# apache/brpc

Hardware: NVIDIA H100
Metric: echo QPS, 1 KB baidu_std (higher is better)
Workload: dtype u8

## Files before the change

### brpc_b200/csrc/b2_api.cu

```cuda
#include <cuda_runtime.h>
#include <dlfcn.h>
#include <stdio.h>
#include <time.h>
#include <stdlib.h>
#include <string.h>
#include <algorithm>
#include <mutex>
#include <string>
#include <unordered_map>
#include <vector>
#include "b2_kernels.cuh"
#include "b2_h2.cuh"

using namespace b2;

static thread_local char g_err[512] = "";
static void set_err(const char* fmt, const char* a = "", const char* b = "") { snprintf(g_err, sizeof g_err, fmt, a, b); }

#define CU(call)                                                                          \
    do {                                                                                  \
        cudaError_t e_ = (call);                                                          \
        if (e_ != cudaSuccess) { set_err("%s: %s", #call, cudaGetErrorString(e_)); return B2_E_CUDA; } \
    } while (0)

namespace {
constexpr int kMaxStages = 16;
constexpr uint32_t kSmallBytes = 128 << 10;
constexpr uint32_t kSmallRuns = 512, kSmallMsgs = 1024;
constexpr size_t kSmallBlock = 64 + kSmallRuns * 32 + kSmallMsgs * (64 + 16) + (kSmallBytes + kSmallMsgs * 80 + 4096);
constexpr uint32_t kSecEvents = 64, kSecMsgs = kSecEvents + kSmallMsgs * 80, kSecCtrl = kSecMsgs + kSmallMsgs * 32,
                   kSecRunCtrl = kSecCtrl + 3 * kStreamCtrlMax * kSmallMsgs, kSecOut = kSecRunCtrl + kSmallRuns * 8;
struct Stage { const char* name; cudaEvent_t ev; };
}

struct b2_ctx {
    b2_options opt;
    DevConfig cfg;
    std::vector<DevMethod> methods;
    uint8_t* d_bytes = nullptr; b2_run* d_runs = nullptr; uint32_t* d_run_tile_base = nullptr;
    TileRec* d_tiles = nullptr; uint32_t* d_tile_base = nullptr; uint32_t* d_tile_scratch = nullptr; uint32_t* d_tile_spec = nullptr; b2_run_status* d_run_status = nullptr;
    uint32_t* d_frame_off = nullptr; uint32_t* d_frame_run = nullptr; b2_msg_desc* d_msgs = nullptr; MsgAux* d_aux = nullptr; PackJob* d_jobs = nullptr; uint32_t* d_slow_idx = nullptr; uint8_t* d_heads = nullptr;
    uint32_t* d_slot = nullptr; uint32_t* d_scan_tmp = nullptr; uint8_t* d_resp = nullptr; uint8_t* d_unz = nullptr; uint16_t* d_snappy_tab = nullptr; HpackState* d_hpack = nullptr; H2Conn* d_h2 = nullptr; H2Stream* d_h2_streams = nullptr; uint8_t* d_h2_slots = nullptr; uint32_t h2_max_conns = B2_H2_MAX_CONNS, h2_pending = B2_H2_MAX_PENDING, h2_stream_bytes = B2_H2_STREAM_BYTES; uint64_t h2_last_in = 0, h2_last_out = 0;
    uint32_t* d_frame_row = nullptr; uint4* d_rows = nullptr;
    std::vector<uint8_t> h2_gunzip; uint8_t* d_h2_gz_merge = nullptr;
    uint8_t* ring_slots = nullptr; volatile uint32_t* ring_ctl = nullptr; uint32_t* d_ring_ticket = nullptr; cudaStream_t ring_stream = nullptr;
    uint32_t ring_next = 1, ring_stride = 0, ring_off_runs = 0, ring_off_in = 0, ring_off_out = 0; bool ring_collected[8] = { true, true, true, true, true, true, true, true };
    const void* ring_bytes[8] = {}; const void* ring_pin_base = nullptr; unsigned long long ring_pin_dev = 0; uint64_t ring_launches = 0;
    bool st_ring = false; StreamPass sp_ring = {}; uint8_t* d_st_ring = nullptr; uint32_t ring_off_st = 0, ring_next_wait = 1, st_view_ticket = 0;
    bool h2_ring = false; uint32_t h2r_max_bytes = 0, h2r_msg_cap = 0, h2r_out_cap = 0, h2r_replies_cap = 0;
    uint32_t h2r_off_args = 0, h2r_off_rs = 0, h2r_off_msgs = 0, h2r_off_spans = 0, h2r_off_out = 0, h2r_off_replies = 0;
    ulonglong2* d_iov = nullptr; b2_iovec* h_iov = nullptr; const void* host_bytes = nullptr;
    uint4* d_refs = nullptr; b2_resp_ref* h_refs = nullptr; int input_mode = B2_INPUT_COPY, resp_mode = B2_RESP_COPY; const uint8_t* pull_bytes = nullptr; uint32_t small_off_refs = 0;
    uint32_t* d_crc_adv = nullptr; unsigned long long* d_counters = nullptr; uint32_t* d_totals = nullptr; DevMethod* d_methods = nullptr;
    size_t meta_tile_off = 0; uint32_t max_tiles = 0; uint32_t n_sms = 132; bool use_tma_pack = true; uint32_t stage_mask = 7;
    StreamPass sp = {}; bool has_streams = false, stream_armed = false, stream_ran = false, stream_valid = false;
    uint32_t st_max = 0, st_open = 0; std::vector<long long> st_keys; std::vector<uint8_t> st_state; std::vector<uint32_t> st_pool, st_pool_free;
    void* d_st_block[10] = {}; void* h_st_mapped[5] = {}; uint32_t* h_st_cnts = nullptr; uint8_t* h_st_out = nullptr; uint8_t* h_st_ctl = nullptr; uint8_t* d_st_ctl = nullptr;
    b2_stream_msg* h_st_msgs = nullptr; b2_stream_event* h_st_events = nullptr; uint8_t* h_st_ctrl = nullptr; uint32_t* h_st_run_ctrl = nullptr;
    cudaEvent_t st_ev[6] = {};
    const uint8_t* st_input = nullptr;
    void* d_sw[4] = {}; size_t sw_have[4] = {}; SwRec* h_sw_recs = nullptr; size_t h_sw_have = 0; uint32_t* h_sw_cnts = nullptr;
    cudaEvent_t sw_ev[8] = {}; bool sw_ran = false;
    b2_run_status* h_run_status = nullptr; b2_msg_desc* h_msgs = nullptr; uint8_t* h_resp = nullptr;
    uint32_t* h_totals = nullptr; uint32_t* h_run_tile_base = nullptr;
    uint32_t n_runs = 0, n_tiles = 0, nbytes = 0, max_run_tiles = 0; uint64_t covered = 0;
    bool uploaded = false, executed = false;
    cudaStream_t stream = nullptr;
    cudaEvent_t ev[kMaxStages + 1];
    const char* stage_names[kMaxStages];
    int n_stages = 0;
    float last_kernel_ms = 0.f; uint32_t last_launches = 0;
    cudaEvent_t ev_first = nullptr, ev_last = nullptr; bool first_pending = true;
    bool profile_stages = false; bool allow_small = true; bool use_fused = true; bool fused_last = false; bool slow_heavy = false;
    bool adaptive_tile = false; bool dense = false; uint32_t avg_frame = 0;
    uint8_t* d_meta = nullptr; uint8_t* h_meta = nullptr;
    uint8_t* d_small = nullptr; uint8_t* h_small = nullptr;
    bool small = false, small_copy_queued = false, use_fused_small = true; uint32_t small_msgs = 0, small_resp = 0, small_off_rs = 0, small_off_msgs = 0, small_off_resp = 0, small_total = 0;
};

static void input_overwritten(b2_ctx* c) { if (c->st_input == c->d_bytes) c->st_input = nullptr; }

static uint32_t g_crc_tab_host[256];
static void crc_table_init() {
    for (uint32_t i = 0; i < 256; i++) {
        uint32_t c = i;
        for (int k = 0; k < 8; k++) c = (c & 1) ? (c >> 1) ^ 0x82f63b78u : (c >> 1);
        g_crc_tab_host[i] = c;
    }
}

extern "C" const char* b2_last_error(void) { return g_err; }
extern "C" const char* b2_version(void) { return "brpc_b200 0.1 (sm_90a)"; }

namespace {
struct BlockPool {
    std::mutex mu;
    static constexpr size_t kSmall = 8192, kSlab = 4u << 20;
    std::vector<uint8_t*> slabs; std::vector<void*> small_free;
    std::unordered_map<void*, int> large_class;
    std::vector<void*> large_free[40];
    uint64_t n_host_alloc = 0;
    void* alloc(size_t size) {
        std::lock_guard<std::mutex> g(mu);
        if (size <= kSmall) {
            if (small_free.empty()) {
                uint8_t* slab = nullptr;
                if (cudaHostAlloc((void**)&slab, kSlab, cudaHostAllocMapped | cudaHostAllocPortable) != cudaSuccess) return nullptr;
                n_host_alloc++; slabs.push_back(slab);
                for (size_t o = 0; o + kSmall <= kSlab; o += kSmall) small_free.push_back(slab + o);
            }
            void* p = small_free.back(); small_free.pop_back(); return p;
        }
        int cls = 14; while (((size_t)1 << cls) < size) cls++;
        if (cls >= 40) return nullptr;
        if (!large_free[cls].empty()) { void* p = large_free[cls].back(); large_free[cls].pop_back(); return p; }
        void* p = nullptr;
        if (cudaHostAlloc(&p, ((size_t)1 << cls) + 1024, cudaHostAllocMapped | cudaHostAllocPortable) != cudaSuccess) return nullptr;
        n_host_alloc++; large_class[p] = cls;
        return p;
    }
    void free(void* p) {
        std::lock_guard<std::mutex> g(mu);
        auto it = large_class.find(p);
        if (it != large_class.end()) { large_free[it->second].push_back(p); return; }
        small_free.push_back(p);
    }
};
BlockPool& block_pool() { static BlockPool* p = new BlockPool; return *p; }
}
extern "C" void* b2_block_alloc(size_t size) {
    void* p = block_pool().alloc(size ? size : 1);
    if (!p) set_err("cudaHostAlloc failed");
    return p;
}
extern "C" void b2_block_free(void* p) { if (p) block_pool().free(p); }
extern "C" uint64_t b2_block_pool_host_allocs(void) { std::lock_guard<std::mutex> g(block_pool().mu); return block_pool().n_host_alloc; }

static void ring_halt(b2_ctx* c);
static void stream_free(b2_ctx* c);
static bool h2_ring_refuses(b2_ctx* c, bool writes_h2_state) {
    if (!c->h2_ring) return false;
    for (uint32_t k = 0; k < kRingSlots; k++) if (!c->ring_collected[k]) { set_err("an h2 ring ticket is outstanding: b2_h2_ring_wait it first"); return true; }
    if (writes_h2_state) ring_halt(c);
    return false;
}
extern "C" void b2_ctx_destroy(b2_ctx* c) {
    if (!c) return;
    cudaSetDevice(c->opt.device);
    ring_halt(c);
    if (c->ring_stream) cudaStreamDestroy(c->ring_stream);
    if (c->ring_slots) cudaFreeHost(c->ring_slots);
    if (c->ring_ctl) cudaFreeHost((void*)c->ring_ctl);
    cudaFree(c->d_ring_ticket);
    cudaFree(c->d_bytes); cudaFree(c->d_runs); cudaFree(c->d_run_tile_base); cudaFree(c->d_tiles); cudaFree(c->d_tile_base); cudaFree(c->d_tile_scratch); cudaFree(c->d_tile_spec);
    cudaFree(c->d_run_status); cudaFree(c->d_frame_off); cudaFree(c->d_frame_run); cudaFree(c->d_msgs); cudaFree(c->d_aux); cudaFree(c->d_jobs); cudaFree(c->d_slow_idx); cudaFree(c->d_heads); cudaFree(c->d_slot);
    cudaFree(c->d_scan_tmp); cudaFree(c->d_resp); cudaFree(c->d_unz); cudaFree(c->d_snappy_tab); cudaFree(c->d_refs); cudaFree(c->d_iov); cudaFreeHost(c->h_iov); cudaFree(c->d_frame_row); cudaFree(c->d_rows); cudaFreeHost(c->h_refs); cudaFree(c->d_hpack); cudaFree(c->d_h2); cudaFree(c->d_h2_streams); cudaFree(c->d_h2_slots); cudaFree(c->d_h2_gz_merge); cudaFree(c->d_counters); cudaFree(c->d_totals); cudaFree(c->d_methods); cudaFree(c->d_crc_adv); cudaFree(c->d_meta); cudaFree(c->d_small); cudaFreeHost(c->h_meta); cudaFreeHost(c->h_small);
    cudaFreeHost(c->h_run_status); cudaFreeHost(c->h_msgs); cudaFreeHost(c->h_resp); cudaFreeHost(c->h_totals);
    cudaFreeHost(c->h_run_tile_base);
    stream_free(c);
    for (int i = 0; i <= kMaxStages; i++) if (c->ev[i]) cudaEventDestroy(c->ev[i]);
    if (c->stream) cudaStreamDestroy(c->stream);
    delete c;
}

extern "C" int b2_ctx_create(const b2_options* o, b2_ctx** out) {
    if (!o || !out) { set_err("null argument"); return B2_E_INVAL; }
    int ndev = 0;
    if (cudaGetDeviceCount(&ndev) != cudaSuccess || ndev == 0) {
        set_err("no CUDA device: brpc_b200 has no CPU path"); return B2_E_NO_DEVICE;
    }
    if (o->device < 0 || o->device >= ndev) { set_err("bad device ordinal"); return B2_E_INVAL; }
    if (o->max_batch_bytes == 0 || o->max_batch_bytes >= (1u << 31) || o->max_msgs == 0 || o->max_runs == 0) {
        set_err("capacities must be non-zero and max_batch_bytes < 2 GiB"); return B2_E_INVAL;
    }
    CU(cudaSetDevice(o->device));
    b2_ctx* c = new b2_ctx();
    { int v = 132; cudaDeviceGetAttribute(&v, cudaDevAttrMultiProcessorCount, o->device); c->n_sms = (uint32_t)v; }
    for (int i = 0; i <= kMaxStages; i++) c->ev[i] = nullptr;
    c->opt = *o;
    c->adaptive_tile = o->tile_bytes == 0;
    uint32_t tile = o->tile_bytes ? o->tile_bytes : 8192;
    if (tile < 512 || (tile & (tile - 1))) { delete c; set_err("tile_bytes must be a power of two >= 512"); return B2_E_INVAL; }
    c->opt.tile_bytes = tile;
    if (c->opt.max_resp_bytes == 0) {
        uint64_t r = (uint64_t)o->max_batch_bytes + (uint64_t)o->max_msgs * 64 + (1u << 20);
        c->opt.max_resp_bytes = r > 0xfffffff0ull ? 0xfffffff0u : (uint32_t)r;
    }
    memset(&c->cfg, 0, sizeof c->cfg);
    c->cfg.max_body_size = o->max_body_size ? o->max_body_size : (64ull << 20);
    c->cfg.proto_mask = kProtoMaskDefault;
    c->cfg.tile_bytes = tile;
    c->cfg.tile_shift = 0; while ((1u << c->cfg.tile_shift) < tile) c->cfg.tile_shift++;
    c->max_tiles = o->max_batch_bytes / tile + o->max_runs + 1;
    const uint32_t scan_blocks = o->max_msgs / (kScanBlock * kScanItems) + 2;
#define ALLOC(ptr, bytes) do { if (cudaMalloc((void**)&(ptr), (bytes)) != cudaSuccess) { set_err("cudaMalloc %s failed", #ptr); b2_ctx_destroy(c); return B2_E_NOMEM; } } while (0)
#define HALLOC(ptr, bytes) do { if (cudaHostAlloc((void**)&(ptr), (bytes), cudaHostAllocDefault) != cudaSuccess) { set_err("cudaHostAlloc %s failed", #ptr); b2_ctx_destroy(c); return B2_E_NOMEM; } } while (0)
    ALLOC(c->d_bytes, (size_t)o->max_batch_bytes + 1024);
    ALLOC(c->d_runs, sizeof(b2_run) * (size_t)o->max_runs);
    ALLOC(c->d_run_tile_base, 4 * ((size_t)o->max_runs + 1));
    ALLOC(c->d_tiles, sizeof(TileRec) * (size_t)c->max_tiles);
    ALLOC(c->d_tile_base, 4 * (size_t)c->max_tiles);
    ALLOC(c->d_tile_scratch, 12 * (size_t)c->max_tiles);
    {
        size_t dense_tiles = (size_t)o->max_batch_bytes / 2048 + o->max_runs + 1; if (dense_tiles > c->max_tiles) dense_tiles = c->max_tiles;
        size_t words = (size_t)kSpecK * c->max_tiles; if ((size_t)kSpecKDense * dense_tiles > words) words = (size_t)kSpecKDense * dense_tiles;
        ALLOC(c->d_tile_spec, 4 * words);
    }
    ALLOC(c->d_run_status, sizeof(b2_run_status) * (size_t)o->max_runs);
    ALLOC(c->d_frame_off, 4 * (size_t)o->max_msgs);
    ALLOC(c->d_frame_run, 4 * (size_t)o->max_msgs);
    ALLOC(c->d_msgs, sizeof(b2_msg_desc) * (size_t)o->max_msgs);
    ALLOC(c->d_aux, sizeof(MsgAux) * (size_t)o->max_msgs);
    ALLOC(c->d_jobs, sizeof(PackJob) * (size_t)o->max_msgs);
    ALLOC(c->d_refs, sizeof(uint4) * (size_t)o->max_msgs);
    ALLOC(c->d_slow_idx, sizeof(uint32_t) * (size_t)o->max_msgs);
    ALLOC(c->d_heads, (size_t)kHeadBytes * (size_t)o->max_msgs);
    ALLOC(c->d_slot, 4 * ((size_t)o->max_msgs + 1));
    ALLOC(c->d_scan_tmp, 4 * (size_t)scan_blocks);
    ALLOC(c->d_resp, (size_t)c->opt.max_resp_bytes + 1024);
    ALLOC(c->d_unz, 2 * (size_t)c->opt.max_resp_bytes + 1024);
    ALLOC(c->d_snappy_tab, (size_t)kSnappyWarps * kSnappyMaxTable * 2);
    ALLOC(c->d_hpack, sizeof(HpackState) * (size_t)B2_HPACK_MAX_CONNS);
    CU(cudaMemset(c->d_hpack, 0, sizeof(HpackState) * (size_t)B2_HPACK_MAX_CONNS));
    ALLOC(c->d_counters, 8 * B2_N_COUNTERS);
    ALLOC(c->d_totals, 64);
    ALLOC(c->d_methods, sizeof(DevMethod) * 64);
    ALLOC(c->d_crc_adv, (kCrcHotWords + kCrcTreeWords) * 4);
    ALLOC(c->d_meta, (size_t)o->max_runs * 28 + 16 * (size_t)c->max_tiles + 64);
    ALLOC(c->d_small, kSmallBlock);
    HALLOC(c->h_meta, (size_t)o->max_runs * 28 + 16 * (size_t)c->max_tiles + 64);
    HALLOC(c->h_small, kSmallBlock);
    HALLOC(c->h_run_status, sizeof(b2_run_status) * (size_t)o->max_runs);
    HALLOC(c->h_msgs, sizeof(b2_msg_desc) * (size_t)o->max_msgs);
    HALLOC(c->h_refs, sizeof(b2_resp_ref) * (size_t)o->max_msgs);
    HALLOC(c->h_resp, (size_t)c->opt.max_resp_bytes);
    HALLOC(c->h_totals, 64);
    HALLOC(c->h_run_tile_base, 4 * ((size_t)o->max_runs + 1));
    CU(cudaMemset(c->d_counters, 0, 8 * B2_N_COUNTERS));
    CU(cudaMemset(c->d_bytes, 0, (size_t)o->max_batch_bytes + 1024));
    CU(cudaStreamCreateWithFlags(&c->stream, cudaStreamNonBlocking));
    for (int i = 0; i <= kMaxStages; i++) CU(cudaEventCreate(&c->ev[i]));
    CU(cudaEventCreate(&c->ev_first)); CU(cudaEventCreate(&c->ev_last));
    crc_table_init();
    CU(cudaMemcpyToSymbol(c_crc_table, g_crc_tab_host, sizeof g_crc_tab_host));
    {
// ... 1696 lines not shown
```

### brpc_b200/csrc/b2_kernels.cuh

```cuda
#pragma once
#include <cuda_runtime.h>
#include "b2_core.cuh"
#include "b2_inflate.cuh"

namespace b2 {

enum TileKind : uint8_t { kRanOff = 0, kStop = 1, kAmbig = 2 };

struct __align__(16) TileRec {
    uint32_t entry;
    uint32_t exit;
    uint32_t count;
    uint8_t kind;
    int8_t last_proto;
    uint8_t live;
    int8_t pf_in;
};

struct __align__(16) MsgAux {
    uint32_t msg_off;
    uint32_t msg_len;
    uint32_t att_len;
    uint32_t att_off;
    uint32_t cks_off;
// ... 1653 lines not shown
#endif
constexpr uint32_t kPackGroup = B2_PACK_GROUP;
constexpr uint32_t kPackGroupSmall = 32;
constexpr uint32_t kStageBytes = B2_STAGE_BYTES;
struct PackWarpSmem {
    alignas(128) uint8_t stage[2][kStageBytes];
    alignas(8) unsigned long long mbar[2];
};

__device__ __forceinline__ uint32_t smem_u32(const void* p) { return (uint32_t)__cvta_generic_to_shared(p); }
__device__ __forceinline__ void mbar_init(unsigned long long* bar, uint32_t count) {
    asm volatile("mbarrier.init.shared::cta.b64 [%0], %1;" ::"r"(smem_u32(bar)), "r"(count) : "memory");
}
__device__ __forceinline__ void mbar_arrive_expect_tx(unsigned long long* bar, uint32_t bytes) {
    asm volatile("mbarrier.arrive.expect_tx.shared::cta.b64 _, [%0], %1;" ::"r"(smem_u32(bar)), "r"(bytes) : "memory");
}
__device__ __forceinline__ void mbar_wait(unsigned long long* bar, uint32_t parity) {
    uint32_t ok;
    do {
        asm volatile("{\n\t.reg .pred p;\n\tmbarrier.try_wait.parity.shared::cta.b64 p, [%1], %2;\n\tselp.u32 %0, 1, 0, p;\n\t}"
                     : "=r"(ok) : "r"(smem_u32(bar)), "r"(parity) : "memory");
    } while (!ok);
}
__device__ __forceinline__ void bulk_g2s(void* sdst, const void* gsrc, uint32_t bytes, unsigned long long* bar) {
    asm volatile("cp.async.bulk.shared::cluster.global.mbarrier::complete_tx::bytes [%0], [%1], %2, [%3];"
                 ::"r"(smem_u32(sdst)), "l"(gsrc), "r"(bytes), "r"(smem_u32(bar)) : "memory");
}
__device__ __forceinline__ void bulk_s2g(void* gdst, const void* ssrc, uint32_t bytes) {
    asm volatile("cp.async.bulk.global.shared::cta.bulk_group [%0], [%1], %2;" ::"l"(gdst), "r"(smem_u32(ssrc)), "r"(bytes) : "memory");
}
__device__ __forceinline__ void bulk_prefetch_l2(const void* gsrc, uint32_t bytes) {
    asm volatile("cp.async.bulk.prefetch.L2.global [%0], %1;" ::"l"(gsrc), "r"(bytes) : "memory");
}
__device__ __forceinline__ void bulk_commit() { asm volatile("cp.async.bulk.commit_group;" ::: "memory"); }
template <int N> __device__ __forceinline__ void bulk_wait_read() { asm volatile("cp.async.bulk.wait_group.read %0;" ::"n"(N) : "memory"); }
template <int N> __device__ __forceinline__ void bulk_wait() { asm volatile("cp.async.bulk.wait_group %0;" ::"n"(N) : "memory"); }

template <uint32_t kGroup>
__global__ void __launch_bounds__(kPackWarps * 32, 1) k_pack_tma(BatchPtrs B, DevConfig C) {
    extern __shared__ __align__(128) uint8_t pack_smem_raw[];
    const uint32_t lane = threadIdx.x & 31, wid = threadIdx.x >> 5;
    PackWarpSmem& S = reinterpret_cast<PackWarpSmem*>(pack_smem_raw)[wid];
    const uint32_t n_msgs = B.totals[0];
    if (B.totals[2] & 3u) return;
    if (lane == 0) {
        mbar_init(&S.mbar[0], 1); mbar_init(&S.mbar[1], 1);
        asm volatile("fence.mbarrier_init.release.cluster;" ::: "memory");
    }
    __syncwarp();
    const uint32_t stride = gridDim.x * kPackWarps * kGroup;
    uint32_t it = 0, phase0 = 0, phase1 = 0;
    PackJob job; job.fast = 0; job.slot_len = 0; job.head_len = 0; job.bulk_len = 0; job.src_off = 0; job.pad = 0;
    uint32_t slot_off = 0;
    uint32_t base = (blockIdx.x * kPackWarps + wid) * kGroup;
    auto fetch = [&](uint32_t bse, PackJob& j, uint32_t& so) {
        const uint32_t i = bse + lane;
        j.fast = 0; j.slot_len = 0;
        if (lane < kGroup && i < n_msgs) {
            const uint4 v = __ldg(reinterpret_cast<const uint4*>(B.jobs + i));
            j = *reinterpret_cast<const PackJob*>(&v);
            so = B.slot[i] + B.scan_tmp[i / (kScanBlock * kScanItems)];
        }
    };
    auto begin_round = [&](uint32_t b) { bulk_wait_read<1>(); __syncwarp(); };
    auto wait_round = [&](uint32_t b) { mbar_wait(&S.mbar[b], (b ? phase1 : phase0) & 1u); if (b) phase1++; else phase0++; };
    if (base < n_msgs) fetch(base, job, slot_off);
    for (; base < n_msgs; base += stride) {
        PackJob njob; uint32_t nslot = 0;
        njob.fast = 0; njob.slot_len = 0; njob.head_len = 0; njob.bulk_len = 0; njob.src_off = 0; njob.pad = 0;
        if (base + stride < n_msgs) fetch(base + stride, njob, nslot);
        uint32_t pending = __ballot_sync(0xffffffffu, job.fast != 0);
        while (pending) {
            const uint32_t b = it & 1; it++;
            uint8_t* stage = S.stage[b];
            const uint32_t first = __ffs(pending) - 1;
            const uint32_t first_len = __shfl_sync(0xffffffffu, job.slot_len, first);
            if (first_len > kStageBytes) {
                const uint32_t hl = __shfl_sync(0xffffffffu, (uint32_t)job.head_len, first);
                const uint32_t so = __shfl_sync(0xffffffffu, slot_off, first);
                const uint32_t src = __shfl_sync(0xffffffffu, job.src_off, first);
                const uint32_t pad = __shfl_sync(0xffffffffu, (uint32_t)job.pad, first);
                const uint8_t* head = B.heads + (size_t)(base + first) * kHeadBytes;
                uint32_t bb = b;
                for (uint32_t c0 = 0; c0 < first_len; c0 += kStageBytes) {
                    const uint32_t c1 = min(c0 + kStageBytes, first_len);
                    if (c0) { bb = it & 1; it++; }
                    uint8_t* st = S.stage[bb];
                    begin_round(bb);
                    if (lane == 0) {
                        mbar_arrive_expect_tx(&S.mbar[bb], c1 - c0);
                        uint32_t at = c0;
                        if (at < hl) { const uint32_t e = min(hl, c1); bulk_g2s(st, head + at, e - at, &S.mbar[bb]); at = e; }
                        if (at < c1) bulk_g2s(st + (at - c0), B.bytes + src + (at - hl), c1 - at, &S.mbar[bb]);
                    }
                    wait_round(bb);
                    if (lane == 0) bulk_s2g(B.resp + so + c0, st, c1 - c0);
                    bulk_commit();
                }
                if (lane == 0) B.msgs[base + first].resp_off = so + pad;
                pending &= ~(1u << first);
                continue;
            }
            const bool mine = (pending >> lane) & 1u;
            uint32_t need = mine ? job.slot_len : 0, incl = need;
            #pragma unroll
            for (int d = 1; d < (int)kGroup; d <<= 1) { const uint32_t y = __shfl_up_sync(0xffffffffu, incl, d); if (lane >= (uint32_t)d) incl += y; }
            const bool take = mine && incl <= kStageBytes;
            const uint32_t soff = incl - need;
            uint32_t tx = take ? (uint32_t)job.head_len + job.bulk_len : 0;
            #pragma unroll
            for (int d = 1; d < (int)kGroup; d <<= 1) tx += __shfl_xor_sync(0xffffffffu, tx, d);
            tx = __shfl_sync(0xffffffffu, tx, 0);
            begin_round(b);
            if (lane == 0) mbar_arrive_expect_tx(&S.mbar[b], tx);
            __syncwarp();
            if (take) {
                bulk_g2s(stage + soff, B.heads + (size_t)(base + lane) * kHeadBytes, job.head_len, &S.mbar[b]);
                if (job.bulk_len) bulk_g2s(stage + soff + job.head_len, B.bytes + job.src_off, job.bulk_len, &S.mbar[b]);
            }
            wait_round(b);
            const uint32_t took = __ballot_sync(0xffffffffu, take);
            if (kGroup > 8) {
                const uint32_t lo = __ffs(took) - 1, span = took >> lo;
                const bool contiguous = took && (span & (span + 1)) == 0;
                uint32_t total = take ? job.slot_len : 0;
                #pragma unroll
                for (int d = 1; d < 32; d <<= 1) total += __shfl_xor_sync(0xffffffffu, total, d);
                if (contiguous) { if (lane == lo) bulk_s2g(B.resp + slot_off, stage + soff, total); }
                else if (take) bulk_s2g(B.resp + slot_off, stage + soff, job.slot_len);
                if (take) B.msgs[base + lane].resp_off = slot_off + job.pad;
            } else if (take) {
                bulk_s2g(B.resp + slot_off, stage + soff, job.slot_len);
                B.msgs[base + lane].resp_off = slot_off + job.pad;
            }
            bulk_commit();
            pending &= ~took;
        }
        job = njob; slot_off = nslot;
    }
    bulk_wait<0>();
}


#ifndef B2_FUSED_BUF
#define B2_FUSED_BUF 10240
#endif
#ifndef B2_FUSED_WARPS
#define B2_FUSED_WARPS 12
#endif
#ifndef B2_FUSED_WARPS_DENSE
#define B2_FUSED_WARPS_DENSE 16
#endif
constexpr uint32_t kFusedWarps = B2_FUSED_WARPS, kFusedWarpsDense = B2_FUSED_WARPS_DENSE, kFusedBuf = B2_FUSED_BUF, kFusedRowStride = 176;
__device__ __forceinline__ bool fused_fast_echo(const BatchPtrs& B, const DevMethod* ms, uint32_t n_ms, uint32_t i, uint32_t fo, uint32_t run_idx,
                                                uint8_t* f, uint32_t avail, uint8_t* pfx_out, DecodeOut& o) {
    if (ld32_any(f) != kMagicPRPC) return false;
    const uint32_t body = __byte_perm(ld32_any(f + 4), 0, 0x0123), meta = __byte_perm(ld32_any(f + 8), 0, 0x0123);
    if (meta < 8 || (uint64_t)12 + meta + 8 > avail || meta > body) return false;
    const uint8_t* m = f + 12; const uint8_t* te = m + meta;
    if (m[0] != 0x0a) return false;
    const uint32_t L = m[1];
    if (L >= 128 || L < 4 || 2 + L > meta) return false;
    const uint8_t* q = m + 2; const uint8_t* e = q + L;
    if (q[0] != 0x0a) return false;
    const uint32_t sl = q[1];
    if (sl >= 128 || sl + 4 > L) return false;
    const uint8_t* svc = q + 2; q = svc + sl;
    if (q[0] != 0x12) return false;
    const uint32_t ml = q[1];
    if (ml >= 128 || (uint32_t)(e - q) < 2 + ml) return false;
    const uint8_t* mth = q + 2; q = mth + ml;
    uint32_t has = B2_HAS_REQUEST; uint64_t v = 0; long long log_id = 0;
    if (q < e) {
        if (*q != 0x18) return false;
        Reader r; r.p = q + 1; r.end = e;
        if (!rd_varint(r, v) || r.p != e) return false;
        log_id = (long long)v; has |= B2_HAS_LOG_ID;
    }
    const uint8_t* t = e;
    if (t + 2 <= te && t[0] == 0x18) { if (t[1] != 0) return false; has |= B2_HAS_COMPRESS_TYPE; t += 2; }
    long long cid = 0;
    if (t < te && t[0] == 0x20) { Reader r; r.p = t + 1; r.end = te; if (!rd_varint(r, v)) return false; cid = (long long)v; has |= B2_HAS_CORRELATION_ID; t = r.p; }
    if (t + 2 <= te && t[0] == 0x50) { if (t[1] != 0) return false; has |= B2_HAS_CONTENT_TYPE; t += 2; }
    if (t + 2 <= te && t[0] == 0x58) { if (t[1] != 0) return false; has |= B2_HAS_CHECKSUM_TYPE; t += 2; }
    if (t + 2 <= te && t[0] == 0x62) { if (t[1] != 0) return false; has |= B2_HAS_CHECKSUM_VALUE; t += 2; }
    if (t != te) return false;
    bool has_dot = false;
    for (uint32_t k = 0; k < sl && !has_dot; k += 4) {
        uint32_t eq = __vcmpeq4(ld32_any(svc + k), 0x2e2e2e2eu);
        if (sl - k < 4) eq &= (1u << (8 * (sl - k))) - 1u;
        has_dot = eq != 0;
    }
    if (!has_dot) return false;
    int idx = -1;
    for (uint32_t k = 0; k < n_ms; k++) {
        const DevMethod& d = ms[k];
        if (d.full_method_len == sl + 1 + ml && d.full_method[sl] == '.' && bytes_eq(svc, d.full_method, sl) && bytes_eq(mth, d.full_method + sl + 1, ml)) { idx = (int)k; break; }
    }
    if (idx < 0) return false;
    const DevMethod& M = ms[idx];
    if (M.handler != B2_HANDLER_ECHO || M.response_checksum_type != B2_CHECKSUM_TYPE_NONE || M.response_compress_type != B2_COMPRESS_TYPE_NONE) return false;
    const uint32_t req_size = body - meta;
    if (req_size < 2 || te[0] != 0x0a) return false;
    Reader r; r.p = te + 1; r.end = te + (req_size < 6 ? req_size : 6);
    if (!rd_varint(r, v)) return false;
    const uint32_t hdr = (uint32_t)(r.p - te);
    if (v > 0x7fffffefull || (uint64_t)hdr + v != req_size) return false;
    const uint32_t msg_len = (uint32_t)v, msg_off = 12 + meta + hdr;
    const uint32_t cidn = varint_len((uint64_t)cid), mlr = 13 + cidn, vl = varint_len(msg_len), prefix = 12 + mlr + 1 + vl;
    if (prefix > msg_off) return false;
    uint8_t* p = pfx_out ? pfx_out : f + msg_off - prefix;
    p[0] = 'P'; p[1] = 'R'; p[2] = 'P'; p[3] = 'C';
    put_be32(p + 4, mlr + 1 + vl + msg_len); put_be32(p + 8, mlr); p += 12;
    p[0] = 0x12; p[1] = 0x02; p[2] = 0x08; p[3] = 0x00; p[4] = 0x18; p[5] = 0x00; p[6] = 0x20; p += 7;
    p = put_varint(p, (uint64_t)cid);
    p[0] = 0x50; p[1] = 0x00; p[2] = 0x58; p[3] = 0x00; p[4] = 0x62; p[5] = 0x00; p[6] = 0x0a; p += 7;
    put_varint(p, msg_len);
    b2_msg_desc d;
    d.run_idx = run_idx; d.frame_off = fo; d.body_size = body; d.meta_size = meta; d.correlation_id = cid; d.log_id = log_id;
    d.attachment_size = 0; d.compress_type = 0; d.checksum_type = 0; d.error_code = 0; d.has_bits = (uint16_t)has; d.protocol = B2_PROTOCOL_BAIDU_STD;
    d.content_type = 0; d.method_idx = (int16_t)idx; d.status = B2_MSG_ECHOED; d.resp_off = fo + msg_off - prefix; d.resp_len = prefix + msg_len;
    B.msgs[i] = d;
    o.fast = true; o.slow = false; o.prefix = prefix; o.rs = d.resp_off;
    return true;
}

struct FusedWarpSmem {
    alignas(128) uint8_t buf[kFusedBuf];
    uint32_t foff[32];
    alignas(8) unsigned long long mbar;
};
__device__ __forceinline__ void fence_proxy_async() { asm volatile("fence.proxy.async.shared::cta;" ::: "memory"); }

__device__ __forceinline__ void fused_store(uint8_t* resp, const uint8_t* img, uint32_t img_off, uint32_t a, uint32_t b, uint32_t lane) {
    if (a >= b) return;
    const uint32_t a0 = (a + 15u) & ~15u, b0 = b & ~15u;
    if (a0 >= b0) { for (uint32_t k = a + lane; k < b; k += 32) resp[k] = img[k - img_off]; return; }
    if (lane == 0) bulk_s2g(resp + a0, img + (a0 - img_off), b0 - a0);
    if (lane < a0 - a) resp[a + lane] = img[a + lane - img_off];
    if (lane >= 16 && lane - 16 < b - b0) resp[b0 + lane - 16] = img[b0 + lane - 16 - img_off];
}

#ifndef B2_FUSED_REGS
#define B2_FUSED_REGS 128
#endif
static_assert(B2_FUSED_REGS * (B2_FUSED_WARPS > B2_FUSED_WARPS_DENSE ? B2_FUSED_WARPS : B2_FUSED_WARPS_DENSE) * 32 <= 65536, "k_fused: registers x threads must fit the SM's register file");
__global__ void __maxnreg__(B2_FUSED_REGS) k_fused(BatchPtrs B, DevConfig C) {
    extern __shared__ __align__(128) uint8_t fused_raw[];
    const uint32_t lane = threadIdx.x & 31, wid = threadIdx.x >> 5;
    FusedWarpSmem& S = reinterpret_cast<FusedWarpSmem*>(fused_raw)[wid];
    if (B.totals[2] & 1u) return;
    __shared__ __align__(16) DevMethod s_methods[2];
    {
        const uint32_t nw = min(C.n_methods, 2u) * (uint32_t)(sizeof(DevMethod) / 4);
        const uint32_t* src = reinterpret_cast<const uint32_t*>(B.methods); uint32_t* dst = reinterpret_cast<uint32_t*>(s_methods);
        for (uint32_t k = threadIdx.x; k < nw; k += blockDim.x) dst[k] = src[k];
    }
    __syncthreads();
    const DevMethod* ms = C.n_methods <= 2 ? s_methods : B.methods;
    if (lane == 0) { mbar_init(&S.mbar, 1); asm volatile("fence.mbarrier_init.release.cluster;" ::: "memory"); }
    __syncwarp();
    uint32_t phase = 0;
    const uint32_t n_warps = gridDim.x * (blockDim.x >> 5);
    uint32_t t = blockIdx.x * (blockDim.x >> 5) + wid;
    uint4 rec_raw = make_uint4(0, 0, 0, 0), ti = make_uint4(0, 0, 0, 0); uint32_t tbase = 0;
    if (t < B.n_tiles) { rec_raw = *reinterpret_cast<const uint4*>(B.tiles + t); ti = __ldg(B.tile_info + t); tbase = B.tile_base[t]; }
    for (; t < B.n_tiles; t += n_warps) {
        const uint4 rec_cur = rec_raw, ti_cur = ti; const uint32_t tbase_cur = tbase;
        const uint32_t tn = t + n_warps;
        if (tn < B.n_tiles) { rec_raw = *reinterpret_cast<const uint4*>(B.tiles + tn); ti = __ldg(B.tile_info + tn); tbase = B.tile_base[tn]; }
        TileRec rec; *reinterpret_cast<uint4*>(&rec) = rec_cur;
        const uint32_t count = rec.count;
        if (!rec.live || count == 0) continue;
        const uint4 ti = ti_cur;
        const uint32_t r = ti.w & 0xffffffu, run_off = ti.x, run_len = ti.y;
        const bool client = ((ti.w >> 24) & B2_RUN_CLIENT) != 0, dump = ((ti.w >> 24) & B2_RUN_RPC_DUMP) != 0;
        const uint32_t first = B.run_status[r].first_msg + tbase_cur;
        const uint32_t hi = run_off + rec.exit;
        const bool spec_ok = !(rec.kind & kKindRewalked) && count <= C.spec_k;
        const uint32_t* spec = B.tile_spec + (size_t)t * C.spec_k;
        uint32_t sub_lo = run_off + rec.entry, wpos = rec.entry; int wpf = rec.pf_in;
        for (uint32_t done = 0; done < count; done += 32) {
            const uint32_t cnt = min(32u, count - done);
            uint32_t fo_raw = 0, sub_hi;
            if (spec_ok) {
                if (lane < cnt) fo_raw = __ldg(spec + done + lane);
                sub_hi = done + cnt < count ? (__ldg(spec + done + cnt) & 0x7fffffffu) : hi;
            } else {
                if (lane == 0) {
                    for (uint32_t k = 0; k < cnt; k++) {
                        const Step sp = cut_input_message(B.bytes + run_off, run_len, wpos, wpf, C.max_body_size, client, run_mask(C.proto_mask, ti.w >> 24));
                        S.foff[k] = (run_off + sp.frame_pos) | ((uint32_t)(sp.index != 1) << 31);
                        wpos = sp.new_pos; wpf = sp.pf;
                    }
                }
                wpos = __shfl_sync(0xffffffffu, wpos, 0); wpf = __shfl_sync(0xffffffffu, wpf, 0);
                __syncwarp();
                if (lane < cnt) fo_raw = S.foff[lane];
                sub_hi = done + cnt < count ? run_off + wpos : hi;
            }
            const uint32_t lo16 = sub_lo & ~15u, hi16 = (sub_hi + 15u) & ~15u, span = hi16 - lo16;
            const uint32_t i = first + done + lane;
            const uint32_t fo = fo_raw & 0x7fffffffu;
            DecodeOut o; o.fast = false; o.slow = false; o.prefix = 0; o.rs = 0;
            const bool fits = span <= kFusedBuf;
            if (fits) {
                if (lane == 0) { bulk_wait_read<0>(); mbar_arrive_expect_tx(&S.mbar, span); bulk_g2s(S.buf, B.bytes + lo16, span, &S.mbar); }
                __syncwarp();
                mbar_wait(&S.mbar, phase & 1u); phase++;
                bool in_place = false;
                if (lane < cnt && i < B.max_msgs) {
                    uint8_t* f = S.buf + (fo - lo16);
                    in_place = !client && !dump && !(fo_raw >> 31) && fused_fast_echo(B, ms, C.n_methods, i, fo, r, f, hi16 - fo, nullptr, o);
                    if (!in_place) decode_one<true>(B, C, i, fo_raw, f, B.heads + (size_t)i * kHeadBytes, 0xffffffffu, r, &o);
                }
                if (in_place) o.prefix = 0;
            } else {
                if (lane == 0) bulk_wait_read<0>();
                __syncwarp();
                const uint32_t sub = lane & 15, half = lane >> 4;
                for (uint32_t m2 = 0; m2 < cnt; m2 += 2) {
                    const uint32_t m = m2 + half;
                    const uint32_t f = __shfl_sync(0xffffffffu, fo, m & 31);
                    if (m < cnt && sub < kRowVecs) {
                        const uint32_t dst = (uint32_t)__cvta_generic_to_shared(S.buf + m * kFusedRowStride + sub * 16);
                        const uint4* src = reinterpret_cast<const uint4*>(B.bytes + (f & ~15u)) + sub;
                        asm volatile("cp.async.cg.shared.global [%0], [%1], 16;" ::"r"(dst), "l"(src) : "memory");
                    }
                }
                asm volatile("cp.async.commit_group;" ::: "memory");
                asm volatile("cp.async.wait_group 0;" ::: "memory");
                __syncwarp();
                if (lane < cnt && i < B.max_msgs) {
                    uint8_t* f = S.buf + lane * kFusedRowStride + (fo & 15u);
                    if (client || dump || (fo_raw >> 31) || !fused_fast_echo(B, ms, C.n_methods, i, fo, r, f, kRowBytes - (fo & 15u), B.heads + (size_t)i * kHeadBytes, o))
                        decode_one<true>(B, C, i, fo_raw, f, B.heads + (size_t)i * kHeadBytes, kRowBytes, r, &o);
                }
                __syncwarp();
            }
            const uint32_t slow_mask = __ballot_sync(0xffffffffu, o.slow);
            if (slow_mask) {
                uint32_t sbase = 0;
                if (lane == 0) sbase = atomicAdd(B.totals + 3, (uint32_t)__popc(slow_mask));
                sbase = __shfl_sync(0xffffffffu, sbase, 0);
                if (o.slow) B.slow_idx[sbase + __popc(slow_mask & ((1u << lane) - 1u))] = i;
            }
            if (fits) {
                if (o.fast && o.prefix) { uint8_t* dst = S.buf + (o.rs - lo16); const uint8_t* src = B.heads + (size_t)i * kHeadBytes; for (uint32_t k = 0; k < o.prefix; k++) dst[k] = src[k]; }
                fence_proxy_async();
                __syncwarp();
                fused_store(B.resp, S.buf, lo16, sub_lo, sub_hi, lane);
                if (lane == 0) bulk_commit();
                __syncwarp();
            } else {
                for (uint32_t c0 = lo16; c0 < hi16; c0 += kFusedBuf) {
                    const uint32_t c1 = min(c0 + kFusedBuf, hi16);
                    if (lane == 0) { bulk_wait_read<0>(); mbar_arrive_expect_tx(&S.mbar, c1 - c0); bulk_g2s(S.buf, B.bytes + c0, c1 - c0, &S.mbar); }
                    __syncwarp();
                    mbar_wait(&S.mbar, phase & 1u); phase++;
                    if (o.fast) {
                        const uint32_t p0 = max(o.rs, c0), p1 = min(o.rs + o.prefix, c1);
                        const uint8_t* pf = B.heads + (size_t)i * kHeadBytes;
                        for (uint32_t k = p0; k < p1; k++) S.buf[k - c0] = pf[k - o.rs];
                    }
                    fence_proxy_async();
                    __syncwarp();
                    fused_store(B.resp, S.buf, c0, max(sub_lo, c0), min(sub_hi, c1), lane);
                    if (lane == 0) bulk_commit();
                    __syncwarp();
                }
            }
            sub_lo = sub_hi;
        }
    }
    if (lane == 0) bulk_wait<0>();
}


struct ReqDesc {
    uint32_t kind, flags; int32_t method_idx, timeout_ms; long long correlation_id, log_id;
    int32_t compress_type, checksum_type, frame_type; uint32_t payload_off, payload_len, attachment_off, attachment_len, reserved;
};
__global__ void __launch_bounds__(256) k_pack_requests(const uint8_t* bytes, const ReqDesc* reqs, uint32_t n, const DevMethod* methods, uint32_t n_methods,
                                                       uint8_t* out, const uint32_t* out_offs, uint32_t* out_lens, uint8_t* scratch,
                                                       uint16_t* snappy_tab, const uint32_t* crc_adv) {
    __shared__ uint32_t s_hot[kCrcHotWords];
    crc_tabs_to_smem(s_hot, crc_adv);
    CrcTabs ct; ct.hot = s_hot; ct.tree = crc_adv + kCrcHotWords;
    const uint32_t lane = threadIdx.x & 31, n_warps = (gridDim.x * blockDim.x) >> 5, warp_id = (blockIdx.x * blockDim.x + threadIdx.x) >> 5;
    for (uint32_t i = warp_id; i < n; i += n_warps) {
        const ReqDesc R = reqs[i];
        uint8_t* o = out + out_offs[i];
        const uint8_t* payload = bytes + R.payload_off;
        if (R.kind == 1) {
            uint8_t meta[40]; uint8_t* m = meta;
            *m++ = 0x08; m = put_varint(m, (uint64_t)R.correlation_id);
            if (R.flags & 1u) { *m++ = 0x10; m = put_varint(m, (uint64_t)R.log_id); }
            *m++ = 0x18; m = put_varint(m, (uint64_t)(long long)R.frame_type);
            if (R.flags & 2u) { *m++ = 0x20; *m++ = (R.flags & 4u) ? 1 : 0; }
            const uint32_t ml = (uint32_t)(m - meta);
            if (lane == 0) {
                o[0] = 'S'; o[1] = 'T'; o[2] = 'R'; o[3] = 'M'; put_be32(o + 4, ml + R.payload_len); put_be32(o + 8, ml);
                for (uint32_t k = 0; k < ml; k++) o[12 + k] = meta[k];
            }
            warp_copy(o + 12 + ml, payload, R.payload_len, lane);
            if (lane == 0) out_lens[i] = 12 + ml + R.payload_len;
            continue;
        }
        if (R.method_idx < 0 || (uint32_t)R.method_idx >= n_methods ||
            (R.compress_type != B2_COMPRESS_TYPE_NONE && R.compress_type != B2_COMPRESS_TYPE_SNAPPY)) { if (lane == 0) out_lens[i] = 0; continue; }
        const DevMethod& M = methods[R.method_idx];
        const uint32_t mth_len = M.full_method_len - M.service_full_len - 1;
        const uint8_t* mth = reinterpret_cast<const uint8_t*>(M.full_method) + M.service_full_len + 1;
        uint32_t rl = 1 + varint_len(M.service_full_len) + M.service_full_len + 1 + varint_len(mth_len) + mth_len;
        if (R.flags & 1u) rl += 1 + varint_len((uint64_t)R.log_id);
        const bool has_to = (R.flags & 2u) && R.timeout_ms > 0;
        if (has_to) rl += 1 + varint_len((uint64_t)(long long)R.timeout_ms);
        const uint32_t cks_len = R.checksum_type == B2_CHECKSUM_TYPE_CRC32C ? 4u : 0u;
        uint32_t ml = 1 + varint_len(rl) + rl + 1 + varint_len((uint64_t)(long long)R.compress_type) + 1 + varint_len((uint64_t)R.correlation_id);
        if (R.attachment_len) ml += 1 + varint_len(R.attachment_len);
        ml += 2 + 1 + varint_len((uint64_t)(long long)R.checksum_type) + 1 + 1 + cks_len;
        uint8_t* body = o + 12 + ml;
        const uint32_t vl = varint_len(R.payload_len), pb_len = 1 + vl + R.payload_len;
        uint32_t body_len;
        if (R.compress_type == B2_COMPRESS_TYPE_SNAPPY) {
            uint8_t* pb = scratch + out_offs[i];
            if (lane == 0) { pb[0] = 0x0a; put_varint(pb + 1, R.payload_len); }
            warp_copy(pb + 1 + vl, payload, R.payload_len, lane);
            __syncwarp();
            body_len = warp_snappy_compress(pb, pb_len, body, snappy_tab + (size_t)(warp_id % kSnappyWarps) * kSnappyMaxTable, lane);
        } else {
            if (lane == 0) { body[0] = 0x0a; put_varint(body + 1, R.payload_len); }
            warp_copy(body + 1 + vl, payload, R.payload_len, lane);
            body_len = pb_len;
        }
        __syncwarp();
        uint32_t crc_be = 0;
        if (cks_len) {
            uint32_t l = 0xffffffffu;
            if (R.compress_type == B2_COMPRESS_TYPE_SNAPPY) { __threadfence_block(); l = warp_crc32c_update(l, body, body_len, lane, ct); }
            else {
                uint8_t hdr[6]; hdr[0] = 0x0a; uint8_t* e = put_varint(hdr + 1, R.payload_len);
                l = crc32c_bytes_serial(l, hdr, (uint32_t)(e - hdr));
                l = warp_crc32c_update(l, payload, R.payload_len, lane, ct);
            }
            crc_be = crc32c_mask(l ^ 0xffffffffu);
        }
        if (R.attachment_len) warp_copy(body + body_len, bytes + R.attachment_off, R.attachment_len, lane);
        if (lane == 0) {
            uint8_t* p = o;
            p[0] = 'P'; p[1] = 'R'; p[2] = 'P'; p[3] = 'C'; put_be32(p + 4, ml + body_len + R.attachment_len); put_be32(p + 8, ml); p += 12;
            *p++ = 0x0a; p = put_varint(p, rl);
            *p++ = 0x0a; p = put_varint(p, M.service_full_len); for (uint32_t k = 0; k < M.service_full_len; k++) *p++ = (uint8_t)M.service_full[k];
            *p++ = 0x12; p = put_varint(p, mth_len); for (uint32_t k = 0; k < mth_len; k++) *p++ = mth[k];
            if (R.flags & 1u) { *p++ = 0x18; p = put_varint(p, (uint64_t)R.log_id); }
            if (has_to) { *p++ = 0x40; p = put_varint(p, (uint64_t)(long long)R.timeout_ms); }
            *p++ = 0x18; p = put_varint(p, (uint64_t)(long long)R.compress_type);
            *p++ = 0x20; p = put_varint(p, (uint64_t)R.correlation_id);
            if (R.attachment_len) { *p++ = 0x28; p = put_varint(p, R.attachment_len); }
            *p++ = 0x50; *p++ = 0x00;
            *p++ = 0x58; p = put_varint(p, (uint64_t)(long long)R.checksum_type);
            *p++ = 0x62; *p++ = (uint8_t)cks_len;
            if (cks_len) p = put_be32(p, crc_be);
            out_lens[i] = 12 + ml + body_len + R.attachment_len;
        }
    }
}

__global__ void __launch_bounds__(256) k_emit_iov(BatchPtrs B, ulonglong2* iov, unsigned long long resp_base, unsigned long long bytes_base) {
    if (B.totals[2] & 3u) return;
    const uint32_t n = B.totals[0];
    for (uint32_t i = blockIdx.x * blockDim.x + threadIdx.x; i < n; i += gridDim.x * blockDim.x) {
        const b2_msg_desc* d = B.msgs + i;
        const uint32_t status = d->status;
        ulonglong2 a = make_ulonglong2(resp_base, 0ull), b = a;
        if (status == B2_MSG_ECHOED || status == B2_MSG_ERROR_REPLIED) {
            const uint4 rf = status == B2_MSG_ECHOED ? B.refs[i] : make_uint4(0, 0, 0, 0);
            a = make_ulonglong2(resp_base + d->resp_off, rf.z ? rf.x : d->resp_len);
            if (rf.z) b = make_ulonglong2(bytes_base + rf.y, rf.z);
        } else atomicAdd(&B.run_status[d->run_idx].n_unanswered, 1u);
        iov[2 * (size_t)i] = a; iov[2 * (size_t)i + 1] = b;
    }
}

struct ReplyDesc {
    uint32_t flags; int32_t error_code; long long correlation_id; int32_t compress_type, checksum_type, content_type;
    uint32_t error_text_off, error_text_len, body_off, body_len, attachment_off, attachment_len, checksum_value_off, checksum_value_len,
             extra_streams_off, n_extra_streams, user_fields_off, n_user_fields, reserved;
    long long stream_id;
};
__device__ __forceinline__ uint32_t reply_user_fields_len(const uint8_t* uf, uint32_t n) {
    uint32_t total = 0;
    for (uint32_t k = 0; k < n; k++) {
        const uint32_t kl = load_le32(uf), vl = load_le32(uf + 4);
        const uint32_t el = 1 + varint_len(kl) + kl + 1 + varint_len(vl) + vl;
        total += 1 + varint_len(el) + el; uf += 8 + kl + vl;
    }
    return total;
}
__global__ void __launch_bounds__(256) k_pack_responses(const uint8_t* bytes, const ReplyDesc* reps, uint32_t n, uint8_t* out, const uint32_t* out_offs,
                                                        uint32_t* out_lens, uint8_t* scratch, uint16_t* snappy_tab, const uint32_t* crc_adv) {
    __shared__ uint32_t s_hot[kCrcHotWords];
    crc_tabs_to_smem(s_hot, crc_adv);
    CrcTabs ct; ct.hot = s_hot; ct.tree = crc_adv + kCrcHotWords;
    const uint32_t lane = threadIdx.x & 31, n_warps = (gridDim.x * blockDim.x) >> 5, warp_id = (blockIdx.x * blockDim.x + threadIdx.x) >> 5;
    for (uint32_t i = warp_id; i < n; i += n_warps) {
        const ReplyDesc R = reps[i];
        uint8_t* o = out + out_offs[i];
        const int32_t err = R.error_code == -1 ? B2_EINTERNAL : R.error_code;
        const bool append_body = err == 0;
        if (append_body && R.compress_type != B2_COMPRESS_TYPE_NONE && R.compress_type != B2_COMPRESS_TYPE_SNAPPY) { if (lane == 0) out_lens[i] = 0; continue; }
        const bool own_cks = append_body && R.checksum_type == B2_CHECKSUM_TYPE_CRC32C;
        const uint32_t cks_len = own_cks ? 4u : R.checksum_value_len;
        const uint32_t att_len = append_body ? R.attachment_len : 0u;
        uint32_t rl = 1 + varint_len((uint64_t)(long long)err);
        if (R.error_text_len) rl += 1 + varint_len(R.error_text_len) + R.error_text_len;
        uint32_t sl = 0;
        const long long* extra = reinterpret_cast<const long long*>(bytes + R.extra_streams_off);
        if (R.flags & B2_RSP_HAS_STREAM) {
            sl = 1 + varint_len((uint64_t)R.stream_id) + 2 + 2;
            for (uint32_t k = 0; k < R.n_extra_streams; k++) sl += 1 + varint_len((uint64_t)extra[k]);
        }
        const uint32_t ufl = R.n_user_fields ? reply_user_fields_len(bytes + R.user_fields_off, R.n_user_fields) : 0u;
        uint32_t ml = 1 + varint_len(rl) + rl + 1 + varint_len((uint64_t)(long long)R.compress_type) + 1 + varint_len((uint64_t)R.correlation_id);
        if (att_len) ml += 1 + varint_len(att_len);
        if (R.flags & B2_RSP_HAS_STREAM) ml += 1 + varint_len(sl) + sl;
        ml += ufl;
        ml += 1 + varint_len((uint64_t)(long long)R.content_type) + 1 + varint_len((uint64_t)(long long)R.checksum_type) + 1 + varint_len(cks_len) + cks_len;
// ... 836 lines not shown
```

Before: 1.009 billion.

## Issue tile bulk load before run-status lookup and add optional phase timers

For speculative tiles with at most 32 messages whose byte span fits the shared buffer, the bulk global-to-shared copy is now issued before the run_status and tile_spec reads. That lets the copy latency overlap with those global loads and the offset setup, and the later fits-path skips reissuing it. The change also adds compile-time-gated clock64 phase instrumentation and a host query function, both off by default. The early issue assumes the span computed from the tile bounds matches the per-chunk span used later.

Result: faster. 1.021 billion, median of 6 (+1.2%).

```diff
diff --git a/brpc_b200/csrc/b2_api.cu b/brpc_b200/csrc/b2_api.cu
--- a/brpc_b200/csrc/b2_api.cu
+++ b/brpc_b200/csrc/b2_api.cu
@@ -91,6 +91,13 @@
 
 extern "C" const char* b2_last_error(void) { return g_err; }
 extern "C" const char* b2_version(void) { return "brpc_b200 0.1 (sm_90a)"; }
+#ifdef B2_FUSED_PHASES
+extern "C" int b2_fused_phases(unsigned long long* out, int reset) {
+    if (cudaDeviceSynchronize() != cudaSuccess || cudaMemcpyFromSymbol(out, g_fused_phases, sizeof(g_fused_phases)) != cudaSuccess) return B2_E_CUDA;
+    if (reset) { static const unsigned long long zero[kFusedPhases] = {}; if (cudaMemcpyToSymbol(g_fused_phases, zero, sizeof(zero)) != cudaSuccess) return B2_E_CUDA; }
+    return B2_OK;
+}
+#endif
 
 namespace {
 struct BlockPool {
diff --git a/brpc_b200/csrc/b2_kernels.cuh b/brpc_b200/csrc/b2_kernels.cuh
--- a/brpc_b200/csrc/b2_kernels.cuh
+++ b/brpc_b200/csrc/b2_kernels.cuh
@@ -1829,8 +1829,21 @@
 #define B2_FUSED_WARPS_DENSE 16
 #endif
 constexpr uint32_t kFusedWarps = B2_FUSED_WARPS, kFusedWarpsDense = B2_FUSED_WARPS_DENSE, kFusedBuf = B2_FUSED_BUF, kFusedRowStride = 176;
+#ifdef B2_FUSED_PHASES
+constexpr uint32_t kFusedPhases = 6;
+__device__ unsigned long long g_fused_phases[kFusedPhases];
+#define B2_PH_STAMP(v) (v) = clock64()
+#define B2_PH_ARG(p) , p
+#else
+#define B2_PH_STAMP(v) ((void)0)
+#define B2_PH_ARG(p)
+#endif
 __device__ __forceinline__ bool fused_fast_echo(const BatchPtrs& B, const DevMethod* ms, uint32_t n_ms, uint32_t i, uint32_t fo, uint32_t run_idx,
-                                                uint8_t* f, uint32_t avail, uint8_t* pfx_out, DecodeOut& o) {
+                                                uint8_t* f, uint32_t avail, uint8_t* pfx_out, DecodeOut& o
+#ifdef B2_FUSED_PHASES
+                                                , long long* t_write = nullptr
+#endif
+                                                ) {
     if (ld32_any(f) != kMagicPRPC) return false;
     const uint32_t body = __byte_perm(ld32_any(f + 4), 0, 0x0123), meta = __byte_perm(ld32_any(f + 8), 0, 0x0123);
     if (meta < 8 || (uint64_t)12 + meta + 8 > avail || meta > body) return false;
@@ -1886,6 +1899,9 @@
     const uint32_t msg_len = (uint32_t)v, msg_off = 12 + meta + hdr;
     const uint32_t cidn = varint_len((uint64_t)cid), mlr = 13 + cidn, vl = varint_len(msg_len), prefix = 12 + mlr + 1 + vl;
     if (prefix > msg_off) return false;
+#ifdef B2_FUSED_PHASES
+    if (t_write) B2_PH_STAMP(*t_write);
+#endif
     uint8_t* p = pfx_out ? pfx_out : f + msg_off - prefix;
     p[0] = 'P'; p[1] = 'R'; p[2] = 'P'; p[3] = 'C';
     put_be32(p + 4, mlr + 1 + vl + msg_len); put_be32(p + 8, mlr); p += 12;
@@ -1938,6 +1954,9 @@
     if (lane == 0) { mbar_init(&S.mbar, 1); asm volatile("fence.mbarrier_init.release.cluster;" ::: "memory"); }
     __syncwarp();
     uint32_t phase = 0;
+#ifdef B2_FUSED_PHASES
+    unsigned long long ph[kFusedPhases] = {}; long long t_prev, t_iss, t_got, t_wr, t_dec, t_end; B2_PH_STAMP(t_prev);
+#endif
     const uint32_t n_warps = gridDim.x * (blockDim.x >> 5);
     uint32_t t = blockIdx.x * (blockDim.x >> 5) + wid;
     uint4 rec_raw = make_uint4(0, 0, 0, 0), ti = make_uint4(0, 0, 0, 0); uint32_t tbase = 0;
@@ -1952,11 +1971,20 @@
         const uint4 ti = ti_cur;
         const uint32_t r = ti.w & 0xffffffu, run_off = ti.x, run_len = ti.y;
         const bool client = ((ti.w >> 24) & B2_RUN_CLIENT) != 0, dump = ((ti.w >> 24) & B2_RUN_RPC_DUMP) != 0;
-        const uint32_t first = B.run_status[r].first_msg + tbase_cur;
         const uint32_t hi = run_off + rec.exit;
         const bool spec_ok = !(rec.kind & kKindRewalked) && count <= C.spec_k;
+        uint32_t sub_lo = run_off + rec.entry, wpos = rec.entry; int wpf = rec.pf_in;
+        bool loaded = false;
+        if (spec_ok && count <= 32u) {
+            const uint32_t lo16 = sub_lo & ~15u, span = ((hi + 15u) & ~15u) - lo16;
+            if (span <= kFusedBuf) {
+                if (lane == 0) { bulk_wait_read<0>(); mbar_arrive_expect_tx(&S.mbar, span); bulk_g2s(S.buf, B.bytes + lo16, span, &S.mbar); }
+                B2_PH_STAMP(t_iss);
+                loaded = true;
+            }
+        }
+        const uint32_t first = B.run_status[r].first_msg + tbase_cur;
         const uint32_t* spec = B.tile_spec + (size_t)t * C.spec_k;
-        uint32_t sub_lo = run_off + rec.entry, wpos = rec.entry; int wpf = rec.pf_in;
         for (uint32_t done = 0; done < count; done += 32) {
             const uint32_t cnt = min(32u, count - done);
             uint32_t fo_raw = 0, sub_hi;
@@ -1982,13 +2010,20 @@
             DecodeOut o; o.fast = false; o.slow = false; o.prefix = 0; o.rs = 0;
             const bool fits = span <= kFusedBuf;
             if (fits) {
-                if (lane == 0) { bulk_wait_read<0>(); mbar_arrive_expect_tx(&S.mbar, span); bulk_g2s(S.buf, B.bytes + lo16, span, &S.mbar); }
+                if (!loaded) {
+                    if (lane == 0) { bulk_wait_read<0>(); mbar_arrive_expect_tx(&S.mbar, span); bulk_g2s(S.buf, B.bytes + lo16, span, &S.mbar); }
+                    B2_PH_STAMP(t_iss);
+                }
                 __syncwarp();
                 mbar_wait(&S.mbar, phase & 1u); phase++;
+                B2_PH_STAMP(t_got);
+#ifdef B2_FUSED_PHASES
+                t_wr = 0;
+#endif
                 bool in_place = false;
                 if (lane < cnt && i < B.max_msgs) {
                     uint8_t* f = S.buf + (fo - lo16);
-                    in_place = !client && !dump && !(fo_raw >> 31) && fused_fast_echo(B, ms, C.n_methods, i, fo, r, f, hi16 - fo, nullptr, o);
+                    in_place = !client && !dump && !(fo_raw >> 31) && fused_fast_echo(B, ms, C.n_methods, i, fo, r, f, hi16 - fo, nullptr, o B2_PH_ARG(&t_wr));
                     if (!in_place) decode_one<true>(B, C, i, fo_raw, f, B.heads + (size_t)i * kHeadBytes, 0xffffffffu, r, &o);
                 }
                 if (in_place) o.prefix = 0;
@@ -2022,6 +2057,7 @@
                 sbase = __shfl_sync(0xffffffffu, sbase, 0);
                 if (o.slow) B.slow_idx[sbase + __popc(slow_mask & ((1u << lane) - 1u))] = i;
             }
+            B2_PH_STAMP(t_dec);
             if (fits) {
                 if (o.fast && o.prefix) { uint8_t* dst = S.buf + (o.rs - lo16); const uint8_t* src = B.heads + (size_t)i * kHeadBytes; for (uint32_t k = 0; k < o.prefix; k++) dst[k] = src[k]; }
                 fence_proxy_async();
@@ -2029,6 +2065,12 @@
                 fused_store(B.resp, S.buf, lo16, sub_lo, sub_hi, lane);
                 if (lane == 0) bulk_commit();
                 __syncwarp();
+#ifdef B2_FUSED_PHASES
+                B2_PH_STAMP(t_end);
+                const long long wr = t_wr ? t_wr : t_dec;
+                ph[0]++; ph[1] += t_iss - t_prev; ph[2] += t_got - t_iss; ph[3] += wr - t_got; ph[4] += t_dec - wr; ph[5] += t_end - t_dec;
+                t_prev = t_end;
+#endif
             } else {
                 for (uint32_t c0 = lo16; c0 < hi16; c0 += kFusedBuf) {
                     const uint32_t c1 = min(c0 + kFusedBuf, hi16);
@@ -2046,11 +2088,15 @@
                     if (lane == 0) bulk_commit();
                     __syncwarp();
                 }
+                B2_PH_STAMP(t_prev);
             }
             sub_lo = sub_hi;
         }
     }
     if (lane == 0) bulk_wait<0>();
+#ifdef B2_FUSED_PHASES
+    if (lane == 0) for (uint32_t k = 0; k < kFusedPhases; k++) atomicAdd(&g_fused_phases[k], ph[k]);
+#endif
 }
 
 
```
